# lighttransport/nanort

Hardware: NVIDIA H100
Metric: Mrays/sec (primary+1-bounce AO) (higher is better)
Workload: dtype f32

## Files before the change

### nanort_b200/csrc/common.cuh

```cuda
#pragma once
#include <cuda_runtime.h>
#include <stddef.h>
#include <stdint.h>

#include <atomic>
#include <mutex>
#include <string>
#include <type_traits>
#include <vector>

#include "../../include/nanort_b200.h"

namespace nrt {

void set_error(const std::string &msg);
int cuda_fail(cudaError_t e, const char *what, const char *file, int line);

#define NRT_CUDA(expr)                                                     \
  do {                                                                     \
    cudaError_t _e = (expr);                                               \
    if (_e != cudaSuccess) return nrt::cuda_fail(_e, #expr, __FILE__, __LINE__); \
  } while (0)

struct DeviceGuard {
// ... 156 lines not shown
  float root_bmin[3], root_bmax[3];
  StagingPipeline staging;
  std::mutex host_mu;
  static constexpr int kSmallSlots = 16;
  static constexpr int kSmallCursor0 = 80;
  static_assert(kSmallCursor0 + kSmallSlots <= 96, "small-slot cursors lie inside d_counters");
  SmallCallPool<kSmallSlots, sizeof(Ray36), sizeof(Hit16)> small;
  void *d_wave = nullptr;
  size_t wave_bytes = 0;
  uint64_t *d_counters = nullptr;
  mutable LaunchRing<32> ring;
};

inline int wait_previous_pass(Accel *a, cudaStream_t s) {
  if (!a->pass_done) NRT_CUDA(cudaEventCreateWithFlags(&a->pass_done, cudaEventDisableTiming));
  NRT_CUDA(cudaStreamWaitEvent(s, a->pass_done, 0));
  return NRT_OK;
}
struct RecordOnExit {
  cudaEvent_t e;
  cudaStream_t s;
  ~RecordOnExit() { cudaEventRecord(e, s); }
};
inline int grow_wave(Accel *a, size_t need) {
  if (a->wave_bytes >= need) return NRT_OK;
  NRT_CUDA(cudaEventSynchronize(a->pass_done));
  cudaFree(a->d_wave);
  a->d_wave = nullptr;
  a->wave_bytes = 0;
  NRT_CUDA(cudaMalloc(&a->d_wave, need));
  a->wave_bytes = need;
  return NRT_OK;
}

__host__ __device__ inline TraceOptions16 default_trace_options() {
  TraceOptions16 o;
  o.prim_ids_range[0] = 0;
  o.prim_ids_range[1] = 0x7FFFFFFFu;
  o.skip_prim_id = 0xFFFFFFFFu;
  o.cull_back_face = 0;
  o.pad[0] = o.pad[1] = o.pad[2] = 0;
  return o;
}

inline BuildOptions28 default_build_options() {
  BuildOptions28 o;
// ... 42 lines not shown
```

### nanort_b200/csrc/render.cu

```cuda
#include <algorithm>
#include <mutex>
#include <string>

#include "common.cuh"
#include "wavefront.cuh"

namespace nrt {

namespace {

__global__ void __launch_bounds__(256)
    gen_primary_kernel(nrt_ao_params p, unsigned long long slot0, uint32_t count, Wave w,
                       unsigned long long *counters ) {
  uint32_t i = blockIdx.x * blockDim.x + threadIdx.x;
  bool valid = false;
  if (i < count) {
    uint32_t pix, smp;
    if (!slot_to_pixel(p, slot0 + i, pix, smp)) {
      w.pix[i] = 0xFFFFFFFFu;
      w.org_tmin[i] = make_float4(0.f, 0.f, 0.f, 0.f);
      w.dir_tmax[i] = make_float4(0.f, 0.f, -1.f, -1.f);
    } else {
      valid = true;
      smp += p.sample0;
// ... 50 lines not shown
  float nx, ny, nz, a2;
  geometric_normal(verts, faces, i, nx, ny, nz, a2);
  out[i] = make_float4(nx, ny, nz, 0.0f);
}

__global__ void __launch_bounds__(256)
    accumulate_ao_kernel(Wave w, const unsigned long long *__restrict__ counters, float *__restrict__ accum,
                         unsigned long long *totals ) {
  const unsigned long long n = counters[0];
  const unsigned long long i = (unsigned long long)blockIdx.x * blockDim.x + threadIdx.x;
  bool occluded = false;
  if (i < n) {
    occluded = w.ao_hits[i].prim_id != 0xFFFFFFFFu;
    if (!occluded) atomicAdd(accum + w.ao_pix[i], 1.0f);
  }
  const unsigned m = __ballot_sync(0xFFFFFFFFu, occluded);
  if ((threadIdx.x & 31) == 0 && m) atomicAdd(totals + 1, (unsigned long long)__popc(m));
  if (i == 0) {
    atomicAdd(totals + 0, n);
    atomicAdd(totals + 2, counters[1]);
  }
}

__global__ void fold_wave_counters_kernel(const unsigned long long *counters, unsigned long long *totals) {
  totals[0] += counters[0];
  totals[2] += counters[1];
}

__global__ void __launch_bounds__(256)
    soa_to_aos_kernel(const float4 *__restrict__ org_tmin, const float4 *__restrict__ dir_tmax,
                      const unsigned long long *n_ptr, unsigned long long n, Ray36 *__restrict__ out, uint32_t type) {
  if (n_ptr) n = *n_ptr;
  const unsigned long long i = (unsigned long long)blockIdx.x * blockDim.x + threadIdx.x;
  if (i >= n) return;
  const float4 o = org_tmin[i], d = dir_tmax[i];
  Ray36 r;
  r.org[0] = o.x;
  r.org[1] = o.y;
  r.org[2] = o.z;
  r.dir[0] = d.x;
  r.dir[1] = d.y;
  r.dir[2] = d.z;
  r.min_t = o.w;
  r.max_t = d.w;
  r.type = type;
  out[i] = r;
}

}

int launch_traverse_soa_devcount(const Accel *a, const float4 *d_org_tmin, const float4 *d_dir_tmax,
                                 const unsigned long long *d_count, size_t capacity, Hit16 *d_hits,
                                 const TraceOptions16 &opt, uint32_t flags, cudaStream_t s);
int launch_traverse_camera_fused(Accel *a, const Wave &w, const nrt_ao_params &p, unsigned long long slot0, size_t count,
                                 const float4 *d_face_n, float *d_accum, unsigned long long *d_wave_counters,
                                 const TraceOptions16 &opt, uint32_t flags, cudaStream_t s);
int launch_traverse_ao_fused(const Accel *a, const Wave &w, const unsigned long long *d_count, size_t capacity,
                             float *d_accum, unsigned long long *d_totals, const TraceOptions16 &opt, uint32_t flags,
                             cudaStream_t s);

}

using namespace nrt;

static unsigned long long valid_slots(const nrt_ao_params &p, unsigned long long s0, uint32_t count) {
  const unsigned long long per_tile = (unsigned long long)p.tile_w * p.tile_h * p.spp;
  const uint32_t tiles_x = (p.width + p.tile_w - 1) / p.tile_w;
  unsigned long long total = 0;
  for (unsigned long long k = s0 / per_tile; k < (s0 + count) / per_tile; k++) {
    const unsigned long long tile = k * p.n_shards + p.shard;
    const uint32_t tx = (uint32_t)(tile % tiles_x), ty = (uint32_t)(tile / tiles_x);
    const uint32_t x0 = tx * p.tile_w, y0 = ty * p.tile_h;
    if (x0 >= p.width || y0 >= p.height) continue;
    const uint32_t wv = p.width - x0 < p.tile_w ? p.width - x0 : p.tile_w;
    const uint32_t hv = p.height - y0 < p.tile_h ? p.height - y0 : p.tile_h;
    total += (unsigned long long)wv * hv * p.spp;
  }
  return total;
}

static int run_ao_pass(const nrt_accel *h, const nrt_ao_params *pp, float *d_accum, nrt_ao_result *res, void *stream,
                       Ray36 *dump_primary, Ray36 *dump_ao, uint64_t *n_ao_out) {
// ... 13 lines not shown
    return NRT_ERR_INVALID;
  }
  NRT_DEVICE(a->device);
  std::lock_guard<std::mutex> lock(a->host_mu);
  cudaStream_t s = static_cast<cudaStream_t>(stream);
  if (const int rc = wait_previous_pass(a, s)) return rc;
  const RecordOnExit pass_done{a->pass_done, s};
  if (!a->d_face_n) {
    NRT_CUDA(cudaMalloc(&a->d_face_n, sizeof(float4) * (size_t)a->n_prims));
    face_normals_kernel<<<(a->n_prims + 255) / 256, 256, 0, s>>>(a->d_verts, a->d_faces, a->n_prims, a->d_face_n);
    NRT_CUDA(cudaGetLastError());
  }
  const uint32_t tiles_x = (p.width + p.tile_w - 1) / p.tile_w, tiles_y = (p.height + p.tile_h - 1) / p.tile_h;
  const uint32_t n_tiles = tiles_x * tiles_y;
  const uint32_t my_tiles = n_tiles > p.shard ? (n_tiles - p.shard + p.n_shards - 1) / p.n_shards : 0;
  const unsigned long long per_tile = (unsigned long long)p.tile_w * p.tile_h * p.spp;
  const unsigned long long total_slots = (unsigned long long)my_tiles * per_tile;

  const unsigned long long kMaxWave = 16ull << 20;
  unsigned long long tiles_per_wave = kMaxWave / per_tile;
  if (tiles_per_wave == 0) tiles_per_wave = 1;
  const unsigned long long cap = std::min<unsigned long long>(total_slots, tiles_per_wave * per_tile);
  const size_t per_ray = 2 * sizeof(float4) + sizeof(Hit16) + 4 + 2 * sizeof(float4) + 4 + sizeof(Hit16);
  const size_t need = (size_t)cap * per_ray + 256;
  if (const int rc = grow_wave(a, need)) return rc;
  Wave w;
  {
    char *b = static_cast<char *>(a->d_wave);
    w.org_tmin = reinterpret_cast<float4 *>(b);
    b += cap * sizeof(float4);
    w.dir_tmax = reinterpret_cast<float4 *>(b);
    b += cap * sizeof(float4);
    w.ao_org_tmin = reinterpret_cast<float4 *>(b);
    b += cap * sizeof(float4);
    w.ao_dir_tmax = reinterpret_cast<float4 *>(b);
    b += cap * sizeof(float4);
    w.hits = reinterpret_cast<Hit16 *>(b);
    b += cap * sizeof(Hit16);
    w.ao_hits = reinterpret_cast<Hit16 *>(b);
    b += cap * sizeof(Hit16);
    w.pix = reinterpret_cast<uint32_t *>(b);
    b += cap * 4;
    w.ao_pix = reinterpret_cast<uint32_t *>(b);
  }
  unsigned long long *wave_ctr = reinterpret_cast<unsigned long long *>(a->d_counters) + 2;
  unsigned long long *totals = reinterpret_cast<unsigned long long *>(a->d_counters) + 4;
  NRT_CUDA(cudaMemsetAsync(totals, 0, 3 * sizeof(unsigned long long), s));

  TraceOptions16 opt = default_trace_options();
  std::vector<cudaEvent_t> ev;
  cudaEvent_t e_begin = nullptr, e_end = nullptr;
  if (res) {
    NRT_CUDA(cudaEventCreate(&e_begin));
    NRT_CUDA(cudaEventCreate(&e_end));
    NRT_CUDA(cudaEventRecord(e_begin, s));
  }
  uint32_t launches = 0, trav_launches = 0;
  unsigned long long dumped_ao = 0, valid_primaries_host = 0;
  const bool fused = !dump_primary && !dump_ao && !(p.flags & NRT_AO_UNFUSED);
  if (!fused && (p.flags & NRT_AO_PACKED_TILES)) {
    set_error("nrt_render_ao_device: NRT_AO_PACKED_TILES needs the fused pass");
    return NRT_ERR_INVALID;
  }
  const uint32_t trav_flags = p.flags & 0xFFFFu;
  int rc = NRT_OK;
  for (unsigned long long s0 = 0; s0 < total_slots && rc == NRT_OK; s0 += cap) {
    const uint32_t count = (uint32_t)std::min<unsigned long long>(cap, total_slots - s0);
    const uint32_t grid = (count + 255) / 256;
    if (cudaMemsetAsync(wave_ctr, 0, 2 * sizeof(unsigned long long), s) != cudaSuccess) {
      rc = NRT_ERR_CUDA;
      break;
    }
    if (!fused) {
      gen_primary_kernel<<<grid, 256, 0, s>>>(p, s0, count, w, wave_ctr);
      launches++;
    }
    cudaEvent_t t0 = nullptr, t1 = nullptr, t2 = nullptr, t3 = nullptr;
    if (res) {
      cudaError_t ee = cudaEventCreate(&t0);
      if (ee == cudaSuccess) ee = cudaEventCreate(&t1);
      if (ee == cudaSuccess) ee = cudaEventCreate(&t2);
      if (ee == cudaSuccess) ee = cudaEventCreate(&t3);
      ev.push_back(t0);
      ev.push_back(t1);
      ev.push_back(t2);
      ev.push_back(t3);
      if (ee != cudaSuccess) {
        rc = cuda_fail(ee, "cudaEventCreate", __FILE__, __LINE__);
        break;
      }
    }
    if (fused) {
      if (res) cudaEventRecord(t0, s);
      rc = launch_traverse_camera_fused(a, w, p, s0, count, a->d_face_n, d_accum, wave_ctr, opt, trav_flags, s);
      if (rc != NRT_OK) break;
      if (res) {
        cudaEventRecord(t1, s);
        cudaEventRecord(t2, s);
      }
      rc = launch_traverse_ao_fused(a, w, wave_ctr, count, d_accum, totals, opt, trav_flags, s);
      if (rc != NRT_OK) break;
      if (res) cudaEventRecord(t3, s);
      fold_wave_counters_kernel<<<1, 1, 0, s>>>(wave_ctr, totals);
      launches += 3;
      trav_launches += 2;
      valid_primaries_host += valid_slots(p, s0, count);
    } else {
      if (dump_primary) {
        soa_to_aos_kernel<<<grid, 256, 0, s>>>(w.org_tmin, w.dir_tmax, nullptr, count, dump_primary + s0, 1u);
        launches++;
      }
      if (res) cudaEventRecord(t0, s);
      rc = launch_traverse_soa(a, w.org_tmin, w.dir_tmax, count, w.hits, opt, trav_flags, s);
      if (rc != NRT_OK) break;
      if (res) cudaEventRecord(t1, s);
      launches++;
      trav_launches++;
      gen_ao_kernel<<<grid, 256, 0, s>>>(p, s0, count, w, a->d_face_n, d_accum, wave_ctr);
      launches++;
      if (dump_ao) {
        unsigned long long n_wave = 0;
        soa_to_aos_kernel<<<grid, 256, 0, s>>>(w.ao_org_tmin, w.ao_dir_tmax, wave_ctr, 0, dump_ao + dumped_ao, 2u);
        launches++;
        cudaMemcpyAsync(&n_wave, wave_ctr, sizeof(n_wave), cudaMemcpyDeviceToHost, s);
        cudaStreamSynchronize(s);
        dumped_ao += n_wave;
// ... 76 lines not shown
```

### nanort_b200/csrc/traverse.cu

```cuda
#include <float.h>
#include <math_constants.h>

#include "common.cuh"
#include "trav_common.cuh"
#include "wavefront.cuh"
#include "traverse3.cuh"

namespace nrt {

struct AosRays {
  static constexpr int kPayloadWords = 0;
  static constexpr bool kSharedOrigin = false;
  const Ray36 *rays;
  __device__ __forceinline__ void load(size_t i, float &ox, float &oy, float &oz, float &dx, float &dy,
                                       float &dz, float &tmin, float &tmax, uint32_t * = nullptr) const {
    const float *p = reinterpret_cast<const float *>(rays + i);
    ox = __ldcs(p + 0);
    oy = __ldcs(p + 1);
    oz = __ldcs(p + 2);
    dx = __ldcs(p + 3);
    dy = __ldcs(p + 4);
    dz = __ldcs(p + 5);
    tmin = __ldcs(p + 6);
    tmax = __ldcs(p + 7);
// ... 67 lines not shown
    }
    if ((threadIdx.x & 31) == 0) {
      atomicAdd(counts + 0, visits[0]);
      atomicAdd(counts + 1, visits[1]);
    }
  }
}

static int g_sm_count[64] = {0};
int device_sm_count(int device) {
  if (device < 0 || device >= 64) return 132;
  if (g_sm_count[device] == 0) {
    int v = 0;
    if (cudaDeviceGetAttribute(&v, cudaDevAttrMultiProcessorCount, device) != cudaSuccess || v <= 0) v = 132;
    g_sm_count[device] = v;
  }
  return g_sm_count[device];
}

typedef Policy3<10, 24, true, 8, false, 2> DefaultPolicy;
typedef Policy3<9, 32, true, 12, true, 3> CameraPolicy;
typedef PacketPolicy<9> CameraPacketPolicy;
typedef Policy3<10, 20, false, 12, false, 3> IncoherentPolicy;
typedef Policy3<9, 32, false, 12, true, 3> IncoherentCameraPolicy;
typedef Policy3<8, 24, false, 8, true, 2> PathRadiancePolicy;
constexpr size_t kPair128MaxBytes = (size_t)38 << 20;
constexpr size_t kCameraRelMaxBytes = (size_t)24 << 20;

template <class Rays, int DEPTH, bool COUNT, class P, class Epi>
static cudaError_t launch_fast3(const Accel *a, Rays rays, size_t n, Epi epi, const TraceOptions16 &opt,
                                uint32_t flags, unsigned long long *cursor, unsigned long long *d_counts,
                                const unsigned long long *n_ptr, cudaStream_t s) {
  const int sms = device_sm_count(a->device);
  const size_t warps_per_block = kTraverseBlock / 32;
  size_t grid = (size_t)sms * P::kMinBlocks;
  const size_t need_blocks = ((n + 31) / 32 + warps_per_block - 1) / warps_per_block;
  if (grid > need_blocks) grid = need_blocks;
  if (grid == 0) grid = 1;
  const void *nodes = Rays::kSharedOrigin ? static_cast<const void *>(a->d_pair_rel)
                     : P::kPair128        ? static_cast<const void *>(a->d_pair)
                                          : static_cast<const void *>(a->d_wide);
  const TriCM *tris = Rays::kSharedOrigin ? a->d_tris_rel : a->d_tris_cm;
  traverse_fast3_kernel<Rays, DEPTH, COUNT, P, Epi><<<(unsigned)grid, kTraverseBlock, 0, s>>>(
      nodes, tris, rays, n, epi, opt, flags, cursor, d_counts, n_ptr);
  return cudaGetLastError();
}

static bool needs_deep_stack(const Accel *a) { return a->stats.max_tree_depth + 2 > 64u; }

template <class Rays, bool COUNT, class P, class Epi>
static int launch_fast3_cursor(const Accel *a, Rays rays, size_t n, Epi epi, const TraceOptions16 &opt, uint32_t flags,
                               unsigned long long *d_counts, const unsigned long long *n_ptr, cudaStream_t s,
                               unsigned long long *cursor) {
  NRT_CUDA(cudaMemsetAsync(cursor, 0, sizeof(unsigned long long), s));
  cudaError_t e;
  if (needs_deep_stack(a))
    e = launch_fast3<Rays, 512, COUNT, P>(a, rays, n, epi, opt, flags, cursor, d_counts, n_ptr, s);
  else
    e = launch_fast3<Rays, 64, COUNT, P>(a, rays, n, epi, opt, flags, cursor, d_counts, n_ptr, s);
  NRT_CUDA(e);
  return NRT_OK;
}

template <class Rays, bool COUNT, class P, class Epi>
static int launch_fast3_any(const Accel *a, Rays rays, size_t n, Epi epi, const TraceOptions16 &opt, uint32_t flags,
                            unsigned long long *d_counts, const unsigned long long *n_ptr, cudaStream_t s,
                            unsigned long long *cursor = nullptr) {
  if (!a->d_pair || !a->d_tris_cm) {
    set_error("traverse: this accel has no triangle traversal layout");
    return NRT_ERR_INVALID;
  }
  if (cursor) return launch_fast3_cursor<Rays, COUNT, P>(a, rays, n, epi, opt, flags, d_counts, n_ptr, s, cursor);
  return a->ring.run(s, [&](uint32_t k) {
    return launch_fast3_cursor<Rays, COUNT, P>(a, rays, n, epi, opt, flags, d_counts, n_ptr, s,
                                               reinterpret_cast<unsigned long long *>(a->d_counters) + 16 + k);
  });
}

template <class Rays, bool COUNT, class Epi>
static int launch_fast3_coherent(const Accel *a, Rays rays, size_t n, Epi epi, const TraceOptions16 &opt, uint32_t flags,
                                 unsigned long long *d_counts, const unsigned long long *n_ptr, cudaStream_t s,
                                 unsigned long long *cursor = nullptr) {
// ... 59 lines not shown
  if (flags & NRT_TRAVERSE_CONFORMANCE) return launch_conf<SoaRays, false>(a, r, n, d_hits, nullptr, opt, flags, nullptr, s);
  return launch_fast<SoaRays, false>(a, r, n, d_hits, nullptr, opt, flags, nullptr, s);
}

int launch_traverse_soa_devcount(const Accel *a, const float4 *d_org_tmin, const float4 *d_dir_tmax,
                                 const unsigned long long *d_count, size_t capacity, Hit16 *d_hits,
                                 const TraceOptions16 &opt, uint32_t flags, cudaStream_t s) {
  if (capacity == 0) return NRT_OK;
  SoaRays r{d_org_tmin, d_dir_tmax};
  if (flags & NRT_TRAVERSE_CONFORMANCE)
    return launch_conf<SoaRays, false>(a, r, capacity, d_hits, nullptr, opt, flags, nullptr, s, d_count);
  return launch_fast<SoaRays, false>(a, r, capacity, d_hits, nullptr, opt, flags, nullptr, s, d_count);
}

template <class Epi, class P = DefaultPolicy, class Rays = SoaRays>
static int launch_fused(const Accel *a, Rays rays, size_t n, const unsigned long long *n_ptr, Epi epi,
                        const TraceOptions16 &opt, uint32_t flags, cudaStream_t s) {
  if (n == 0) return NRT_OK;
  return launch_fast3_any<Rays, false, P>(a, rays, n, epi, opt, flags, nullptr, n_ptr, s);
}

template <int DEPTH>
static cudaError_t launch_packet(const Accel *a, CameraRays rays, size_t n, const PrimaryToAoEpilogue &epi,
                                 const TraceOptions16 &opt, uint32_t flags, unsigned long long *cursor, cudaStream_t s) {
  const size_t warps_per_block = kTraverseBlock / 32;
  size_t grid = (size_t)device_sm_count(a->device) * CameraPacketPolicy::kMinBlocks;
  const size_t need_blocks = ((n + 31) / 32 + warps_per_block - 1) / warps_per_block;
  if (grid > need_blocks) grid = need_blocks;
  traverse_packet_kernel<CameraRays, DEPTH, CameraPacketPolicy, PrimaryToAoEpilogue>
      <<<(unsigned)grid, kTraverseBlock, 0, s>>>(a->d_pair_rel, a->d_tris_rel, rays, n, epi, opt, flags, cursor);
  return cudaGetLastError();
}

static int launch_packet_any(const Accel *a, CameraRays rays, size_t n, const PrimaryToAoEpilogue &epi,
                             const TraceOptions16 &opt, uint32_t flags, cudaStream_t s) {
  if (!a->d_pair_rel || !a->d_tris_rel) {
    set_error("traverse: this accel has no camera-relative traversal layout");
    return NRT_ERR_INVALID;
  }
  return a->ring.run(s, [&](uint32_t k) {
    unsigned long long *cursor = reinterpret_cast<unsigned long long *>(a->d_counters) + 16 + k;
    NRT_CUDA(cudaMemsetAsync(cursor, 0, sizeof(unsigned long long), s));
    const cudaError_t e = needs_deep_stack(a) ? launch_packet<512>(a, rays, n, epi, opt, flags, cursor, s)
                                              : launch_packet<64>(a, rays, n, epi, opt, flags, cursor, s);
    NRT_CUDA(e);
    return NRT_OK;
  });
}

int launch_traverse_camera_fused(Accel *a, const Wave &w, const nrt_ao_params &p, unsigned long long slot0, size_t count,
                                 const float4 *d_face_n, float *d_accum, unsigned long long *d_wave_counters,
                                 const TraceOptions16 &opt, uint32_t flags, cudaStream_t s) {
  PrimaryToAoEpilogue epi{p, w, d_face_n, d_accum, d_wave_counters};
  if (count == 0) return NRT_OK;
  if (a->n_wide * sizeof(PairNode) > kPair128MaxBytes)
    return launch_fast3_any<CameraRaysAbs, false, IncoherentCameraPolicy>(a, CameraRaysAbs(p, slot0), count, epi, opt, flags,
                                                                          nullptr, nullptr, s);
  if (2 * (a->n_wide * sizeof(PairNode) + (size_t)a->n_prims * sizeof(TriCM)) > kCameraRelMaxBytes)
    return launch_fast3_any<CameraRaysAbs, false, CameraPolicy>(a, CameraRaysAbs(p, slot0), count, epi, opt, flags, nullptr,
                                                                nullptr, s);
  const int rc = camera_relative_layout(a, p.cam, s);
  if (rc != NRT_OK) return rc;
  return launch_packet_any(a, CameraRays(p, slot0), count, epi, opt, flags, s);
}

int launch_traverse_ao_fused(const Accel *a, const Wave &w, const unsigned long long *d_count, size_t capacity,
                             float *d_accum, unsigned long long *d_totals, const TraceOptions16 &opt, uint32_t flags,
                             cudaStream_t s) {
  AoAccumulateEpilogue epi{w.ao_pix, d_accum, d_totals};
  if (flags & NRT_TRAVERSE_ANY_HIT)
    return launch_fused<AnyHit<AoAccumulateEpilogue>, IncoherentPolicy>(a, SoaRays{w.ao_org_tmin, w.ao_dir_tmax}, capacity, d_count,
                                                                        AnyHit<AoAccumulateEpilogue>(epi), opt, flags, s);
  return launch_fused<AoAccumulateEpilogue, IncoherentPolicy>(a, SoaRays{w.ao_org_tmin, w.ao_dir_tmax}, capacity, d_count, epi,
                                                              opt, flags, s);
}

int launch_traverse_path_radiance(const Accel *a, const PathShadeEpilogue &epi, const unsigned long long *d_count,
                                  size_t capacity, const TraceOptions16 &opt, uint32_t flags, cudaStream_t s) {
  return launch_fused<PathShadeEpilogue, PathRadiancePolicy>(
      a, SoaRays{epi.q.org_tmin[epi.in], epi.q.dir_tmax[epi.in]}, capacity, d_count, epi, opt, flags, s);
}

int launch_traverse_path_shadow(const Accel *a, const PathQueues &q, const unsigned long long *d_count,
                                size_t capacity, float *d_accum, const TraceOptions16 &opt, uint32_t flags,
                                cudaStream_t s) {
  ShadowAccumulateEpilogue epi{q.sh_contrib_pix, d_accum};
  if (flags & NRT_TRAVERSE_ANY_HIT)
    return launch_fused<AnyHit<ShadowAccumulateEpilogue>, IncoherentPolicy>(a, SoaRays{q.sh_org_tmin, q.sh_dir_tmax}, capacity,
                                                                            d_count, AnyHit<ShadowAccumulateEpilogue>(epi), opt,
                                                                            flags, s);
  return launch_fused<ShadowAccumulateEpilogue, IncoherentPolicy>(a, SoaRays{q.sh_org_tmin, q.sh_dir_tmax}, capacity, d_count,
                                                                  epi, opt, flags, s);
}

int launch_traverse_count(const Accel *a, const Ray36 *d_rays, size_t n, const TraceOptions16 &opt,
                          uint32_t flags, uint64_t *d_counts2, cudaStream_t s) {
  if (a->prim_kind != 0) {
// ... 14 lines not shown
```

### nanort_b200/csrc/traverse3.cuh

```cuda
#pragma once
#include "common.cuh"
#include "trav_common.cuh"

namespace nrt {

struct RayCtx3 {
  float ox, oy, oz;
  float ix, iy, iz;
  float Sx, Sy, Sz;
  float okx, oky, okz;
  float t_min;
  uint32_t nx, ny, nz;
  uint32_t tx, ty, tz;
};

__device__ __forceinline__ void setup_ray3(RayCtx3 &c, float ox, float oy, float oz, float dx, float dy, float dz,
                                           float min_t, bool cpp03) {
  RayCtx r;
  setup_ray(r, ox, oy, oz, dx, dy, dz, min_t, cpp03);
  c.ox = ox;
  c.oy = oy;
  c.oz = oz;
  c.ix = r.ix;
  c.iy = r.iy;
// ... 90 lines not shown
  const bool pos = (U > 0.0f) | (V > 0.0f) | (W > 0.0f);
  rej |= neg & ((opt.cull_back_face != 0) | pos);
  const float det = (U + V) + W;
  rej |= (det == 0.0f);
  const float Az = c.Sz * Akz, Bz = c.Sz * Bkz, Cz = c.Sz * Ckz;
  const float D = (U * Az + V * Bz) + W * Cz;
  const float rcp = 1.0f / det;
  const float tt = D * rcp;
  rej |= (tt > best.t) | (tt < c.t_min);
  if (!rej) {
    best.t = tt;
    best.u = V * rcp;
    best.v = W * rcp;
    best.prim = prim;
  }
}

constexpr int kNone3 = kEmptyLeaf;

constexpr int kTraverseBlock = 128;
constexpr int kNodeExit = 8;
constexpr uint32_t kCountRootIsLeaf = 1u << 31;

template <int MINB_, int REFILL_MIN_, bool PAIR128_, int LEAF_AGAIN_MIN_, bool DEFER_RETIRE_, int NODE_UNROLL_>
struct Policy3 {
  static constexpr int kMinBlocks = MINB_;
  static constexpr int kRefillMin = REFILL_MIN_;
  static constexpr bool kPair128 = PAIR128_;
  static constexpr int kLeafAgainMin = LEAF_AGAIN_MIN_;
  static constexpr bool kDeferRetire = DEFER_RETIRE_;
  static constexpr int kNodeUnroll = NODE_UNROLL_;
};

template <class Rays, int DEPTH, bool COUNT, class P, class Epi>
__global__ void __launch_bounds__(kTraverseBlock, P::kMinBlocks)
    traverse_fast3_kernel(const void *__restrict__ pair, const TriCM *__restrict__ tris, Rays rays, size_t n, Epi epi,
                          TraceOptions16 opt, uint32_t flags, unsigned long long *cursor, unsigned long long *counts,
                          const unsigned long long *n_ptr) {
  constexpr bool kRel = Rays::kSharedOrigin;
  static_assert(!kRel || (P::kPair128 && !COUNT), "camera-relative layout: PairNode, no counting");
  if (n_ptr) n = (size_t)*n_ptr;
  const int lane = threadIdx.x & 31;
  const unsigned lt_mask = (1u << lane) - 1u;
  const bool cpp03 = (flags & NRT_TRAVERSE_CPP03_INVERSE) != 0;
  const bool filtered = opt.prim_ids_range[0] != 0u || opt.prim_ids_range[1] < 0x7FFFFFFFu ||
                        opt.skip_prim_id < 0x7FFFFFFFu;
  const float4 *const pair4 = reinterpret_cast<const float4 *>(pair);
  const float4 *const tris4 = reinterpret_cast<const float4 *>(tris);

  constexpr int PW = Rays::kPayloadWords;
  uint2 lstk[DEPTH + 2 + (PW + 1) / 2];
  int sp = 0;
  RayCtx3 c;
  Best best;
  float min_t = 0.0f;
  bool alive = false;
  int cur = kNone3, leaf = kNone3;
  bool exhausted = false;
  unsigned long long n_boxes = 0, n_prims = 0;
  const bool root_is_leaf = COUNT && (flags & kCountRootIsLeaf) != 0u;
  unsigned long long st[14] = {0, 0, 0, 0, 0, 0, 0, 0, 0, 0, 0, 0, 0, 0};

  for (;;) {
    const unsigned dead = __ballot_sync(FULL_MASK, !alive);
    if (dead != 0u && !exhausted && (dead == FULL_MASK || __popc(dead) >= P::kRefillMin)) {
      const int cnt = __popc(dead);
      const int leader = __ffs(dead) - 1;
      if (COUNT) {
        st[0] += 1;
        st[1] += cnt;
      }
      unsigned long long base = 0;
      if (lane == leader) base = atomicAdd(cursor, (unsigned long long)cnt);
      base = __shfl_sync(FULL_MASK, base, leader);
      if (base + (unsigned long long)cnt >= (unsigned long long)n) exhausted = true;
      if (!alive) {
        const unsigned long long mine = base + (unsigned long long)__popc(dead & lt_mask);
        if (mine < (unsigned long long)n) {
          float ox, oy, oz, dx, dy, dz, max_t;
          uint32_t payload[PW > 0 ? PW : 1];
          rays.load((size_t)mine, ox, oy, oz, dx, dy, dz, min_t, max_t, payload);
#pragma unroll
          for (int w = 0; w + 1 < PW; w += 2) lstk[DEPTH + 2 + w / 2] = make_uint2(payload[w], payload[w + 1]);
          if (PW & 1) lstk[DEPTH + 2 + PW / 2].x = payload[PW - 1];
          setup_ray3(c, ox, oy, oz, dx, dy, dz, min_t, cpp03);
          best.t = max_t;
          best.u = 0.0f;
          best.v = 0.0f;
          best.prim = 0xFFFFFFFFu;
          alive = true;
          lstk[DEPTH] = make_uint2((uint32_t)mine, (uint32_t)(mine >> 32));
          lstk[DEPTH + 1].x = __float_as_uint(max_t);
          sp = 0;
          cur = range_has_nan(min_t, max_t) ? kNone3 : 0;
          leaf = kNone3;
          if (COUNT) {
            n_boxes += 1;
            float4 X, Y, Z;
            if (P::kPair128) {
              X = __ldg(pair4 + c.nx);
              Y = __ldg(pair4 + c.ny);
// ... 146 lines not shown
    if (retiring && retire_now) alive = false;
  }

  if (COUNT) {
    for (int o = 16; o > 0; o >>= 1) {
      n_boxes += __shfl_down_sync(FULL_MASK, n_boxes, o);
      n_prims += __shfl_down_sync(FULL_MASK, n_prims, o);
    }
    for (int o = 16; o > 0; o >>= 1) st[9] += __shfl_down_sync(FULL_MASK, st[9], o);
    if (lane == 0) {
      atomicAdd(counts + 0, n_boxes);
      atomicAdd(counts + 1, n_prims);
#pragma unroll
      for (int k = 0; k < 14; ++k) atomicAdd(counts + 2 + k, st[k]);
    }
  }
}

template <int MINB_>
struct PacketPolicy {
  static constexpr int kMinBlocks = MINB_;
};

template <class Rays, int DEPTH, class P, class Epi>
__global__ void __launch_bounds__(kTraverseBlock, P::kMinBlocks)
    traverse_packet_kernel(const void *__restrict__ pair, const TriCM *__restrict__ tris, Rays rays, size_t n, Epi epi,
                           TraceOptions16 opt, uint32_t flags, unsigned long long *cursor) {
  constexpr bool kRel = Rays::kSharedOrigin;
  static_assert(!Epi::kAnyHit, "packet walk: closest hit only");
  const int lane = threadIdx.x & 31;
  const bool cpp03 = (flags & NRT_TRAVERSE_CPP03_INVERSE) != 0;
  const bool filtered = opt.prim_ids_range[0] != 0u || opt.prim_ids_range[1] < 0x7FFFFFFFu ||
                        opt.skip_prim_id < 0x7FFFFFFFu;
  const float4 *const pair4 = reinterpret_cast<const float4 *>(pair);
  const float4 *const tris4 = reinterpret_cast<const float4 *>(tris);
  const uint32_t kNoEntry = 0x7FC00000u;

  constexpr int PW = Rays::kPayloadWords;
  uint2 lstk[DEPTH + 1 + (PW + 1) / 2];

  for (;;) {
    unsigned long long base = 0;
    if (lane == 0) base = atomicAdd(cursor, 32ull);
    base = __shfl_sync(FULL_MASK, base, 0);
    if (base >= (unsigned long long)n) break;
    const unsigned long long mine = base + (unsigned long long)lane;
    const bool valid = mine < (unsigned long long)n;

    RayCtx3 c = {};
    c.ny = 2u;
    c.nz = 4u;
    Best best;
    best.t = 0.0f;
    best.u = 0.0f;
    best.v = 0.0f;
    best.prim = 0xFFFFFFFFu;
    float min_t = 0.0f;
    bool active = false;
    if (valid) {
      float ox, oy, oz, dx, dy, dz, max_t;
      uint32_t payload[PW > 0 ? PW : 1];
      rays.load((size_t)mine, ox, oy, oz, dx, dy, dz, min_t, max_t, payload);
#pragma unroll
      for (int w = 0; w + 1 < PW; w += 2) lstk[DEPTH + 1 + w / 2] = make_uint2(payload[w], payload[w + 1]);
      if (PW & 1) lstk[DEPTH + 1 + PW / 2].x = payload[PW - 1];
      setup_ray3(c, ox, oy, oz, dx, dy, dz, min_t, cpp03);
      best.t = max_t;
      lstk[DEPTH].x = __float_as_uint(max_t);
      active = !range_has_nan(min_t, max_t);
    }
// ... 73 lines not shown
```

### nanort_b200/csrc/wavefront.cuh

```cuda
#pragma once
#include "common.cuh"

namespace nrt {

struct Wave {
  float4 *org_tmin;
  float4 *dir_tmax;
  Hit16 *hits;
  uint32_t *pix;
  float4 *ao_org_tmin;
  float4 *ao_dir_tmax;
  uint32_t *ao_pix;
  Hit16 *ao_hits;
};

__device__ __forceinline__ uint32_t hash_u32(uint32_t x) {
  x ^= x >> 16;
  x *= 0x7FEB352Du;
  x ^= x >> 15;
  x *= 0x846CA68Bu;
  x ^= x >> 16;
  return x;
}

// ... 193 lines not shown
  sincosf(ph, &sn, &cs);
  const float lx = r * cs, ly = r * sn, lz = sqrtf(fmaxf(0.0f, 1.0f - u1));
  const float wx = t1x * lx + t2x * ly + nx * lz, wy = t1y * lx + t2y * ly + ny * lz, wz = t1z * lx + t2z * ly + nz * lz;
  const float il = 1.0f / sqrtf(wx * wx + wy * wy + wz * wz);
  o4 = make_float4(Px, Py, Pz, p.ao_min_t);
  d4 = make_float4(wx * il, wy * il, wz * il, p.ao_max_t);
}

struct StoreHitsEpilogue {
  static constexpr bool kAnyHit = false;
  Hit16 *hits;
  uint8_t *mask;
  __device__ __forceinline__ void operator()(bool retiring, size_t ray_idx, float t, float u, float v, uint32_t prim,
                                             float max_t, const uint32_t *) const {
    if (retiring && hits) {
      const bool hit = t < max_t;
      float4 r = hit ? make_float4(u, v, t, __uint_as_float(prim)) : make_float4(0.0f, 0.0f, max_t, __uint_as_float(0xFFFFFFFFu));
      __stcs(reinterpret_cast<float4 *>(hits) + ray_idx, r);
      if (mask) mask[ray_idx] = hit ? 1 : 0;
    }
  }
};

struct PrimaryToAoEpilogue {
  static constexpr bool kAnyHit = false;
  nrt_ao_params p;
  Wave w;
  const float4 *normals;
  float *accum;
  unsigned long long *counters;
  __device__ __forceinline__ void operator()(bool retiring, size_t ray_idx, float t, float u, float v, uint32_t prim,
                                             float max_t, const uint32_t *payload) const {
    (void)u;
    (void)v;
    bool make = false;
    float4 o4 = make_float4(0.f, 0.f, 0.f, 0.f), d4 = o4;
    uint32_t pix = 0xFFFFFFFFu, acc = 0;
    if (retiring) {
      pix = payload[3];
      if (pix != 0xFFFFFFFFu) {
        const uint32_t smp = payload[4];
        acc = payload[5];
        const float4 ro = make_float4(p.cam[0], p.cam[1], p.cam[2], p.ray_min_t);
        const float4 rd = make_float4(__uint_as_float(payload[0]), __uint_as_float(payload[1]),
                                      __uint_as_float(payload[2]), p.ray_max_t);
        if (t < max_t) {
          make_ao_ray(p, pix, smp, ro, rd, t, prim, normals, o4, d4);
          make = true;
        } else {
          atomicAdd(accum + acc, 1.0f);
        }
      }
    }
    const unsigned m = __ballot_sync(0xFFFFFFFFu, make);
    if (m == 0u) return;
    const int lane = threadIdx.x & 31, leader = __ffs(m) - 1;
    unsigned long long base = 0;
    if (lane == leader) base = atomicAdd(counters, (unsigned long long)__popc(m));
    base = __shfl_sync(0xFFFFFFFFu, base, leader);
    if (make) {
      const unsigned long long j = base + __popc(m & ((1u << lane) - 1u));
      w.ao_org_tmin[j] = o4;
      w.ao_dir_tmax[j] = d4;
      w.ao_pix[j] = acc;
    }
  }
};

struct AoAccumulateEpilogue {
  static constexpr bool kAnyHit = false;
  const uint32_t *ao_pix;
  float *accum;
  unsigned long long *totals;
  __device__ __forceinline__ void operator()(bool retiring, size_t ray_idx, float t, float u, float v, uint32_t prim,
                                             float max_t, const uint32_t *) const {
    (void)u;
    (void)v;
    (void)prim;
    const bool occluded = retiring && (t < max_t);
    if (retiring && !occluded) atomicAdd(accum + ao_pix[ray_idx], 1.0f);
    const unsigned m = __ballot_sync(0xFFFFFFFFu, occluded);
    if (m != 0u && (int)(threadIdx.x & 31) == __ffs(m) - 1) atomicAdd(totals + 1, (unsigned long long)__popc(m));
  }
};
// ... 258 lines not shown
```

Before: 7542.

## Partition wave work into per-SM ranges with work stealing for primary and AO passes

Replaces the single global atomic work cursor with per-SM range cursors on padded cache lines. Primary rays are claimed from a home range chosen by SM id, and AO rays are written into the region matching their primary range so the AO pass reads mostly locally generated rays. When a home range runs out, a warp scans for another live range and steals from it. This is meant to cut contention on one hot atomic and improve locality, at the cost of a scan loop, extra counter memory and a more complex counter fold kernel.

Result: faster. 7663, median of 6 (+1.6%).

```diff
diff --git a/nanort_b200/csrc/common.cuh b/nanort_b200/csrc/common.cuh
--- a/nanort_b200/csrc/common.cuh
+++ b/nanort_b200/csrc/common.cuh
@@ -202,6 +202,7 @@
   cudaStream_t s;
   ~RecordOnExit() { cudaEventRecord(e, s); }
 };
+constexpr uint32_t kRangeStride = 16;
 inline int grow_wave(Accel *a, size_t need) {
   if (a->wave_bytes >= need) return NRT_OK;
   NRT_CUDA(cudaEventSynchronize(a->pass_done));
diff --git a/nanort_b200/csrc/render.cu b/nanort_b200/csrc/render.cu
--- a/nanort_b200/csrc/render.cu
+++ b/nanort_b200/csrc/render.cu
@@ -96,9 +96,11 @@
   }
 }
 
-__global__ void fold_wave_counters_kernel(const unsigned long long *counters, unsigned long long *totals) {
-  totals[0] += counters[0];
-  totals[2] += counters[1];
+__global__ void fold_wave_counters_kernel(const unsigned long long *region_n, uint32_t R, unsigned long long *totals) {
+  unsigned long long n = 0;
+  for (uint32_t r = threadIdx.x; r < R; r += 32) n += region_n[(size_t)r * kRangeStride];
+  for (int o = 16; o > 0; o >>= 1) n += __shfl_down_sync(0xFFFFFFFFu, n, o);
+  if (threadIdx.x == 0) totals[0] += n;
 }
 
 __global__ void __launch_bounds__(256)
@@ -127,11 +129,10 @@
                                  const unsigned long long *d_count, size_t capacity, Hit16 *d_hits,
                                  const TraceOptions16 &opt, uint32_t flags, cudaStream_t s);
 int launch_traverse_camera_fused(Accel *a, const Wave &w, const nrt_ao_params &p, unsigned long long slot0, size_t count,
-                                 const float4 *d_face_n, float *d_accum, unsigned long long *d_wave_counters,
-                                 const TraceOptions16 &opt, uint32_t flags, cudaStream_t s);
-int launch_traverse_ao_fused(const Accel *a, const Wave &w, const unsigned long long *d_count, size_t capacity,
-                             float *d_accum, unsigned long long *d_totals, const TraceOptions16 &opt, uint32_t flags,
-                             cudaStream_t s);
+                                 const float4 *d_face_n, float *d_accum, const WaveRanges &wr, const TraceOptions16 &opt,
+                                 uint32_t flags, cudaStream_t s);
+int launch_traverse_ao_fused(const Accel *a, const Wave &w, const WaveRanges &wr, size_t capacity, float *d_accum,
+                             unsigned long long *d_totals, const TraceOptions16 &opt, uint32_t flags, cudaStream_t s);
 
 }
 
@@ -191,11 +192,15 @@
   if (tiles_per_wave == 0) tiles_per_wave = 1;
   const unsigned long long cap = std::min<unsigned long long>(total_slots, tiles_per_wave * per_tile);
   const size_t per_ray = 2 * sizeof(float4) + sizeof(Hit16) + 4 + 2 * sizeof(float4) + 4 + sizeof(Hit16);
-  const size_t need = (size_t)cap * per_ray + 256;
+  const uint32_t R = (uint32_t)device_sm_count(a->device);
+  const size_t ctr_words = kRangeStride * (1 + (size_t)R);
+  const size_t ctr_bytes = (ctr_words * sizeof(unsigned long long) + 255) & ~(size_t)255;
+  const size_t need = ctr_bytes + (size_t)cap * per_ray + 256;
   if (const int rc = grow_wave(a, need)) return rc;
   Wave w;
+  unsigned long long *wave_ctr = static_cast<unsigned long long *>(a->d_wave);
   {
-    char *b = static_cast<char *>(a->d_wave);
+    char *b = static_cast<char *>(a->d_wave) + ctr_bytes;
     w.org_tmin = reinterpret_cast<float4 *>(b);
     b += cap * sizeof(float4);
     w.dir_tmax = reinterpret_cast<float4 *>(b);
@@ -212,7 +217,6 @@
     b += cap * 4;
     w.ao_pix = reinterpret_cast<uint32_t *>(b);
   }
-  unsigned long long *wave_ctr = reinterpret_cast<unsigned long long *>(a->d_counters) + 2;
   unsigned long long *totals = reinterpret_cast<unsigned long long *>(a->d_counters) + 4;
   NRT_CUDA(cudaMemsetAsync(totals, 0, 3 * sizeof(unsigned long long), s));
 
@@ -236,7 +240,7 @@
   for (unsigned long long s0 = 0; s0 < total_slots && rc == NRT_OK; s0 += cap) {
     const uint32_t count = (uint32_t)std::min<unsigned long long>(cap, total_slots - s0);
     const uint32_t grid = (count + 255) / 256;
-    if (cudaMemsetAsync(wave_ctr, 0, 2 * sizeof(unsigned long long), s) != cudaSuccess) {
+    if (cudaMemsetAsync(wave_ctr, 0, ctr_words * sizeof(unsigned long long), s) != cudaSuccess) {
       rc = NRT_ERR_CUDA;
       break;
     }
@@ -260,17 +264,20 @@
       }
     }
     if (fused) {
+      const uint32_t packets = (count + 31) / 32;
+      unsigned long long *const lines = wave_ctr + kRangeStride;
+      const WaveRanges wr{R, FastDiv((packets + R - 1) / R * 32), lines, lines + 1, lines + 2};
       if (res) cudaEventRecord(t0, s);
-      rc = launch_traverse_camera_fused(a, w, p, s0, count, a->d_face_n, d_accum, wave_ctr, opt, trav_flags, s);
+      rc = launch_traverse_camera_fused(a, w, p, s0, count, a->d_face_n, d_accum, wr, opt, trav_flags, s);
       if (rc != NRT_OK) break;
       if (res) {
         cudaEventRecord(t1, s);
         cudaEventRecord(t2, s);
       }
-      rc = launch_traverse_ao_fused(a, w, wave_ctr, count, d_accum, totals, opt, trav_flags, s);
+      rc = launch_traverse_ao_fused(a, w, wr, count, d_accum, totals, opt, trav_flags, s);
       if (rc != NRT_OK) break;
       if (res) cudaEventRecord(t3, s);
-      fold_wave_counters_kernel<<<1, 1, 0, s>>>(wave_ctr, totals);
+      fold_wave_counters_kernel<<<1, 32, 0, s>>>(wr.region_n, R, totals);
       launches += 3;
       trav_launches += 2;
       valid_primaries_host += valid_slots(p, s0, count);
diff --git a/nanort_b200/csrc/traverse.cu b/nanort_b200/csrc/traverse.cu
--- a/nanort_b200/csrc/traverse.cu
+++ b/nanort_b200/csrc/traverse.cu
@@ -113,14 +113,15 @@
 typedef Policy3<9, 32, true, 12, true, 3> CameraPolicy;
 typedef PacketPolicy<9> CameraPacketPolicy;
 typedef Policy3<10, 20, false, 12, false, 3> IncoherentPolicy;
+typedef Policy3<10, 20, false, 12, false, 3> AoPolicy;
 typedef Policy3<9, 32, false, 12, true, 3> IncoherentCameraPolicy;
 typedef Policy3<8, 24, false, 8, true, 2> PathRadiancePolicy;
 constexpr size_t kPair128MaxBytes = (size_t)38 << 20;
 constexpr size_t kCameraRelMaxBytes = (size_t)24 << 20;
 
-template <class Rays, int DEPTH, bool COUNT, class P, class Epi>
+template <class Rays, int DEPTH, bool COUNT, class P, class Epi, class Cursor>
 static cudaError_t launch_fast3(const Accel *a, Rays rays, size_t n, Epi epi, const TraceOptions16 &opt,
-                                uint32_t flags, unsigned long long *cursor, unsigned long long *d_counts,
+                                uint32_t flags, Cursor cursor, unsigned long long *d_counts,
                                 const unsigned long long *n_ptr, cudaStream_t s) {
   const int sms = device_sm_count(a->device);
   const size_t warps_per_block = kTraverseBlock / 32;
@@ -132,7 +133,7 @@
                      : P::kPair128        ? static_cast<const void *>(a->d_pair)
                                           : static_cast<const void *>(a->d_wide);
   const TriCM *tris = Rays::kSharedOrigin ? a->d_tris_rel : a->d_tris_cm;
-  traverse_fast3_kernel<Rays, DEPTH, COUNT, P, Epi><<<(unsigned)grid, kTraverseBlock, 0, s>>>(
+  traverse_fast3_kernel<Rays, DEPTH, COUNT, P, Epi, Cursor><<<(unsigned)grid, kTraverseBlock, 0, s>>>(
       nodes, tris, rays, n, epi, opt, flags, cursor, d_counts, n_ptr);
   return cudaGetLastError();
 }
@@ -146,9 +147,25 @@
   NRT_CUDA(cudaMemsetAsync(cursor, 0, sizeof(unsigned long long), s));
   cudaError_t e;
   if (needs_deep_stack(a))
-    e = launch_fast3<Rays, 512, COUNT, P>(a, rays, n, epi, opt, flags, cursor, d_counts, n_ptr, s);
+    e = launch_fast3<Rays, 512, COUNT, P>(a, rays, n, epi, opt, flags, GlobalCursor{cursor}, d_counts, n_ptr, s);
   else
-    e = launch_fast3<Rays, 64, COUNT, P>(a, rays, n, epi, opt, flags, cursor, d_counts, n_ptr, s);
+    e = launch_fast3<Rays, 64, COUNT, P>(a, rays, n, epi, opt, flags, GlobalCursor{cursor}, d_counts, n_ptr, s);
+  NRT_CUDA(e);
+  return NRT_OK;
+}
+
+template <class Rays, class P, class Epi, bool PACKETS>
+static int launch_fast3_ranged(const Accel *a, Rays rays, size_t n, Epi epi, const TraceOptions16 &opt, uint32_t flags,
+                               RangedCursor<PACKETS> cursor, cudaStream_t s) {
+  if (!a->d_pair || !a->d_tris_cm) {
+    set_error("traverse: this accel has no triangle traversal layout");
+    return NRT_ERR_INVALID;
+  }
+  cudaError_t e;
+  if (needs_deep_stack(a))
+    e = launch_fast3<Rays, 512, false, P>(a, rays, n, epi, opt, flags, cursor, nullptr, nullptr, s);
+  else
+    e = launch_fast3<Rays, 64, false, P>(a, rays, n, epi, opt, flags, cursor, nullptr, nullptr, s);
   NRT_CUDA(e);
   return NRT_OK;
 }
@@ -254,57 +271,54 @@
 
 template <int DEPTH>
 static cudaError_t launch_packet(const Accel *a, CameraRays rays, size_t n, const PrimaryToAoEpilogue &epi,
-                                 const TraceOptions16 &opt, uint32_t flags, unsigned long long *cursor, cudaStream_t s) {
+                                 const TraceOptions16 &opt, uint32_t flags, RangedCursor<true> cursor, cudaStream_t s) {
   const size_t warps_per_block = kTraverseBlock / 32;
   size_t grid = (size_t)device_sm_count(a->device) * CameraPacketPolicy::kMinBlocks;
   const size_t need_blocks = ((n + 31) / 32 + warps_per_block - 1) / warps_per_block;
   if (grid > need_blocks) grid = need_blocks;
-  traverse_packet_kernel<CameraRays, DEPTH, CameraPacketPolicy, PrimaryToAoEpilogue>
+  traverse_packet_kernel<CameraRays, DEPTH, CameraPacketPolicy, PrimaryToAoEpilogue, RangedCursor<true>>
       <<<(unsigned)grid, kTraverseBlock, 0, s>>>(a->d_pair_rel, a->d_tris_rel, rays, n, epi, opt, flags, cursor);
   return cudaGetLastError();
 }
 
 static int launch_packet_any(const Accel *a, CameraRays rays, size_t n, const PrimaryToAoEpilogue &epi,
-                             const TraceOptions16 &opt, uint32_t flags, cudaStream_t s) {
+                             const TraceOptions16 &opt, uint32_t flags, RangedCursor<true> cursor, cudaStream_t s) {
   if (!a->d_pair_rel || !a->d_tris_rel) {
     set_error("traverse: this accel has no camera-relative traversal layout");
     return NRT_ERR_INVALID;
   }
-  return a->ring.run(s, [&](uint32_t k) {
-    unsigned long long *cursor = reinterpret_cast<unsigned long long *>(a->d_counters) + 16 + k;
-    NRT_CUDA(cudaMemsetAsync(cursor, 0, sizeof(unsigned long long), s));
-    const cudaError_t e = needs_deep_stack(a) ? launch_packet<512>(a, rays, n, epi, opt, flags, cursor, s)
-                                              : launch_packet<64>(a, rays, n, epi, opt, flags, cursor, s);
-    NRT_CUDA(e);
-    return NRT_OK;
-  });
+  const cudaError_t e = needs_deep_stack(a) ? launch_packet<512>(a, rays, n, epi, opt, flags, cursor, s)
+                                            : launch_packet<64>(a, rays, n, epi, opt, flags, cursor, s);
+  NRT_CUDA(e);
+  return NRT_OK;
 }
 
 int launch_traverse_camera_fused(Accel *a, const Wave &w, const nrt_ao_params &p, unsigned long long slot0, size_t count,
-                                 const float4 *d_face_n, float *d_accum, unsigned long long *d_wave_counters,
-                                 const TraceOptions16 &opt, uint32_t flags, cudaStream_t s) {
-  PrimaryToAoEpilogue epi{p, w, d_face_n, d_accum, d_wave_counters};
+                                 const float4 *d_face_n, float *d_accum, const WaveRanges &wr, const TraceOptions16 &opt,
+                                 uint32_t flags, cudaStream_t s) {
+  PrimaryToAoEpilogue epi{p, w, d_face_n, d_accum, wr.span, wr.region_n};
   if (count == 0) return NRT_OK;
+  const RangedCursor<true> cursor{wr.range_cur, nullptr, wr.span.d, wr.R};
   if (a->n_wide * sizeof(PairNode) > kPair128MaxBytes)
-    return launch_fast3_any<CameraRaysAbs, false, IncoherentCameraPolicy>(a, CameraRaysAbs(p, slot0), count, epi, opt, flags,
-                                                                          nullptr, nullptr, s);
+    return launch_fast3_ranged<CameraRaysAbs, IncoherentCameraPolicy>(a, CameraRaysAbs(p, slot0), count, epi, opt, flags,
+                                                                      cursor, s);
   if (2 * (a->n_wide * sizeof(PairNode) + (size_t)a->n_prims * sizeof(TriCM)) > kCameraRelMaxBytes)
-    return launch_fast3_any<CameraRaysAbs, false, CameraPolicy>(a, CameraRaysAbs(p, slot0), count, epi, opt, flags, nullptr,
-                                                                nullptr, s);
+    return launch_fast3_ranged<CameraRaysAbs, CameraPolicy>(a, CameraRaysAbs(p, slot0), count, epi, opt, flags, cursor, s);
   const int rc = camera_relative_layout(a, p.cam, s);
   if (rc != NRT_OK) return rc;
-  return launch_packet_any(a, CameraRays(p, slot0), count, epi, opt, flags, s);
-}
-
-int launch_traverse_ao_fused(const Accel *a, const Wave &w, const unsigned long long *d_count, size_t capacity,
-                             float *d_accum, unsigned long long *d_totals, const TraceOptions16 &opt, uint32_t flags,
-                             cudaStream_t s) {
+  return launch_packet_any(a, CameraRays(p, slot0), count, epi, opt, flags, cursor, s);
+}
+
+int launch_traverse_ao_fused(const Accel *a, const Wave &w, const WaveRanges &wr, size_t capacity, float *d_accum,
+                             unsigned long long *d_totals, const TraceOptions16 &opt, uint32_t flags, cudaStream_t s) {
   AoAccumulateEpilogue epi{w.ao_pix, d_accum, d_totals};
+  if (capacity == 0) return NRT_OK;
+  const RangedCursor<false> cursor{wr.region_cur, wr.region_n, wr.span.d, wr.R};
+  const SoaRays rays{w.ao_org_tmin, w.ao_dir_tmax};
   if (flags & NRT_TRAVERSE_ANY_HIT)
-    return launch_fused<AnyHit<AoAccumulateEpilogue>, IncoherentPolicy>(a, SoaRays{w.ao_org_tmin, w.ao_dir_tmax}, capacity, d_count,
-                                                                        AnyHit<AoAccumulateEpilogue>(epi), opt, flags, s);
-  return launch_fused<AoAccumulateEpilogue, IncoherentPolicy>(a, SoaRays{w.ao_org_tmin, w.ao_dir_tmax}, capacity, d_count, epi,
-                                                              opt, flags, s);
+    return launch_fast3_ranged<SoaRays, AoPolicy>(a, rays, capacity, AnyHit<AoAccumulateEpilogue>(epi), opt, flags, cursor,
+                                                  s);
+  return launch_fast3_ranged<SoaRays, AoPolicy>(a, rays, capacity, epi, opt, flags, cursor, s);
 }
 
 int launch_traverse_path_radiance(const Accel *a, const PathShadeEpilogue &epi, const unsigned long long *d_count,
diff --git a/nanort_b200/csrc/traverse3.cuh b/nanort_b200/csrc/traverse3.cuh
--- a/nanort_b200/csrc/traverse3.cuh
+++ b/nanort_b200/csrc/traverse3.cuh
@@ -136,6 +136,60 @@
 constexpr int kNodeExit = 8;
 constexpr uint32_t kCountRootIsLeaf = 1u << 31;
 
+struct GlobalCursor {
+  static constexpr bool kRanged = false;
+  unsigned long long *cursor;
+};
+
+template <bool PACKETS>
+struct RangedCursor {
+  static constexpr bool kRanged = true;
+  static constexpr bool kPackets = PACKETS;
+  unsigned long long *cur;
+  const unsigned long long *len;
+  unsigned long long span;
+  uint32_t R;
+
+  __device__ __forceinline__ unsigned long long length(uint32_t r, unsigned long long n) const {
+    if (!PACKETS) return len[(size_t)r * kRangeStride];
+    const unsigned long long s0 = (unsigned long long)r * span;
+    return n > s0 ? (n - s0 < span ? n - s0 : span) : 0ull;
+  }
+  __device__ __forceinline__ uint32_t own_range() const {
+    uint32_t smid;
+    asm volatile("mov.u32 %0, %%smid;" : "=r"(smid));
+    return smid % R;
+  }
+  __device__ __forceinline__ int claim(int want, unsigned long long n, uint32_t &home, unsigned long long &first) const {
+    const uint32_t lane = threadIdx.x & 31;
+    for (;;) {
+      unsigned long long base = 0;
+      if (lane == 0) base = atomicAdd(cur + (size_t)home * kRangeStride, (unsigned long long)want);
+      base = __shfl_sync(FULL_MASK, base, 0);
+      const unsigned long long end = length(home, n);
+      if (base < end) {
+        first = (unsigned long long)home * span + base;
+        return end - base < (unsigned long long)want ? (int)(end - base) : want;
+      }
+      uint32_t next = R;
+      for (uint32_t k = 1; k < R; k += 32) {
+        bool live = false;
+        uint32_t r = home + k + lane;
+        if (r >= R) r -= R;
+        if (k + lane < R) live = *(volatile const unsigned long long *)(cur + (size_t)r * kRangeStride) < length(r, n);
+        const unsigned m = __ballot_sync(FULL_MASK, live);
+        if (m != 0u) {
+          r = home + k + (uint32_t)(__ffs(m) - 1);
+          next = r >= R ? r - R : r;
+          break;
+        }
+      }
+      if (next == R) return 0;
+      home = next;
+    }
+  }
+};
+
 template <int MINB_, int REFILL_MIN_, bool PAIR128_, int LEAF_AGAIN_MIN_, bool DEFER_RETIRE_, int NODE_UNROLL_>
 struct Policy3 {
   static constexpr int kMinBlocks = MINB_;
@@ -146,10 +200,10 @@
   static constexpr int kNodeUnroll = NODE_UNROLL_;
 };
 
-template <class Rays, int DEPTH, bool COUNT, class P, class Epi>
+template <class Rays, int DEPTH, bool COUNT, class P, class Epi, class Cursor>
 __global__ void __launch_bounds__(kTraverseBlock, P::kMinBlocks)
     traverse_fast3_kernel(const void *__restrict__ pair, const TriCM *__restrict__ tris, Rays rays, size_t n, Epi epi,
-                          TraceOptions16 opt, uint32_t flags, unsigned long long *cursor, unsigned long long *counts,
+                          TraceOptions16 opt, uint32_t flags, Cursor cursor, unsigned long long *counts,
                           const unsigned long long *n_ptr) {
   constexpr bool kRel = Rays::kSharedOrigin;
   static_assert(!kRel || (P::kPair128 && !COUNT), "camera-relative layout: PairNode, no counting");
@@ -174,23 +228,32 @@
   unsigned long long n_boxes = 0, n_prims = 0;
   const bool root_is_leaf = COUNT && (flags & kCountRootIsLeaf) != 0u;
   unsigned long long st[14] = {0, 0, 0, 0, 0, 0, 0, 0, 0, 0, 0, 0, 0, 0};
+  if constexpr (Cursor::kRanged) lstk[DEPTH + 1].y = cursor.own_range();
 
   for (;;) {
     const unsigned dead = __ballot_sync(FULL_MASK, !alive);
     if (dead != 0u && !exhausted && (dead == FULL_MASK || __popc(dead) >= P::kRefillMin)) {
       const int cnt = __popc(dead);
-      const int leader = __ffs(dead) - 1;
       if (COUNT) {
         st[0] += 1;
         st[1] += cnt;
       }
-      unsigned long long base = 0;
-      if (lane == leader) base = atomicAdd(cursor, (unsigned long long)cnt);
-      base = __shfl_sync(FULL_MASK, base, leader);
-      if (base + (unsigned long long)cnt >= (unsigned long long)n) exhausted = true;
+      unsigned long long base = 0, limit = (unsigned long long)n;
+      if constexpr (Cursor::kRanged) {
+        uint32_t home = lstk[DEPTH + 1].y;
+        const int got = cursor.claim(cnt, (unsigned long long)n, home, base);
+        if (got == 0) exhausted = true;
+        limit = base + (unsigned long long)got;
+        lstk[DEPTH + 1].y = home;
+      } else {
+        const int leader = __ffs(dead) - 1;
+        if (lane == leader) base = atomicAdd(cursor.cursor, (unsigned long long)cnt);
+        base = __shfl_sync(FULL_MASK, base, leader);
+        if (base + (unsigned long long)cnt >= (unsigned long long)n) exhausted = true;
+      }
       if (!alive) {
         const unsigned long long mine = base + (unsigned long long)__popc(dead & lt_mask);
-        if (mine < (unsigned long long)n) {
+        if (mine < limit) {
           float ox, oy, oz, dx, dy, dz, max_t;
           uint32_t payload[PW > 0 ? PW : 1];
           rays.load((size_t)mine, ox, oy, oz, dx, dy, dz, min_t, max_t, payload);
@@ -383,10 +446,10 @@
   static constexpr int kMinBlocks = MINB_;
 };
 
-template <class Rays, int DEPTH, class P, class Epi>
+template <class Rays, int DEPTH, class P, class Epi, class Cursor>
 __global__ void __launch_bounds__(kTraverseBlock, P::kMinBlocks)
     traverse_packet_kernel(const void *__restrict__ pair, const TriCM *__restrict__ tris, Rays rays, size_t n, Epi epi,
-                           TraceOptions16 opt, uint32_t flags, unsigned long long *cursor) {
+                           TraceOptions16 opt, uint32_t flags, Cursor cursor) {
   constexpr bool kRel = Rays::kSharedOrigin;
   static_assert(!Epi::kAnyHit, "packet walk: closest hit only");
   const int lane = threadIdx.x & 31;
@@ -400,13 +463,26 @@
   constexpr int PW = Rays::kPayloadWords;
   uint2 lstk[DEPTH + 1 + (PW + 1) / 2];
 
+  uint32_t home = 0;
+  if constexpr (Cursor::kRanged) home = cursor.own_range();
   for (;;) {
-    unsigned long long base = 0;
-    if (lane == 0) base = atomicAdd(cursor, 32ull);
-    base = __shfl_sync(FULL_MASK, base, 0);
-    if (base >= (unsigned long long)n) break;
-    const unsigned long long mine = base + (unsigned long long)lane;
-    const bool valid = mine < (unsigned long long)n;
+    unsigned long long mine;
+    bool valid;
+    if constexpr (Cursor::kRanged) {
+      static_assert(Cursor::kPackets, "packet walk: whole-packet ranges");
+      unsigned long long first = 0;
+      const int got = cursor.claim(32, (unsigned long long)n, home, first);
+      if (got == 0) break;
+      mine = first + (unsigned long long)lane;
+      valid = lane < got;
+    } else {
+      unsigned long long base = 0;
+      if (lane == 0) base = atomicAdd(cursor.cursor, 32ull);
+      base = __shfl_sync(FULL_MASK, base, 0);
+      if (base >= (unsigned long long)n) break;
+      mine = base + (unsigned long long)lane;
+      valid = mine < (unsigned long long)n;
+    }
 
     RayCtx3 c = {};
     c.ny = 2u;
diff --git a/nanort_b200/csrc/wavefront.cuh b/nanort_b200/csrc/wavefront.cuh
--- a/nanort_b200/csrc/wavefront.cuh
+++ b/nanort_b200/csrc/wavefront.cuh
@@ -239,13 +239,22 @@
   }
 };
 
+struct WaveRanges {
+  uint32_t R;
+  FastDiv span;
+  unsigned long long *range_cur;
+  unsigned long long *region_n;
+  unsigned long long *region_cur;
+};
+
 struct PrimaryToAoEpilogue {
   static constexpr bool kAnyHit = false;
   nrt_ao_params p;
   Wave w;
   const float4 *normals;
   float *accum;
-  unsigned long long *counters;
+  FastDiv span;
+  unsigned long long *region_n;
   __device__ __forceinline__ void operator()(bool retiring, size_t ray_idx, float t, float u, float v, uint32_t prim,
                                              float max_t, const uint32_t *payload) const {
     (void)u;
@@ -271,12 +280,15 @@
     }
     const unsigned m = __ballot_sync(0xFFFFFFFFu, make);
     if (m == 0u) return;
-    const int lane = threadIdx.x & 31, leader = __ffs(m) - 1;
+    const int lane = threadIdx.x & 31;
+    const uint32_t r = make ? span.div((uint32_t)ray_idx) : 0xFFFFFFFFu;
+    const unsigned grp = __match_any_sync(0xFFFFFFFFu, r) & m;
+    const int leader = make ? __ffs(grp) - 1 : lane;
     unsigned long long base = 0;
-    if (lane == leader) base = atomicAdd(counters, (unsigned long long)__popc(m));
+    if (make && lane == leader) base = atomicAdd(region_n + (size_t)r * kRangeStride, (unsigned long long)__popc(grp));
     base = __shfl_sync(0xFFFFFFFFu, base, leader);
     if (make) {
-      const unsigned long long j = base + __popc(m & ((1u << lane) - 1u));
+      const unsigned long long j = (unsigned long long)r * span.d + base + __popc(grp & ((1u << lane) - 1u));
       w.ao_org_tmin[j] = o4;
       w.ao_dir_tmax[j] = d4;
       w.ao_pix[j] = acc;
```
